# mit-acl/dpgo_ros

Measured on AMD Instinct MI355X. Metric: ms/RBCD-iteration + iterations-to-1e-6-relcost, sphere2500 5-agent, lower is better.
Workload: dtype f64; 1 GPU; sphere2500.g2o, 5 agents, synchronous round-robin RBCD, RGD(step 0.2, dense preconditioner) + Nesterov (restart 20), r=5, library weighting; mid-run iterations one launch each (k_step_fd: the private part of an agent's preconditioner product formed by the launch before its own, its row products by the one before that), hipGraphs of up to 256 iterations; agents=5, poses_per_agent=500, placement=agent a on rank a % N

## Files before the change

dpgo_ros_amd/csrc/device_math.h:

```cpp
#pragma once
#include <hip/hip_runtime.h>

namespace dpgo {

typedef double v2d_t __attribute__((ext_vector_type(2)));

template <class T>
__device__ __forceinline__ __attribute__((address_space(1))) T *gp(T *p) { return (__attribute__((address_space(1))) T *)p; }

__device__ __forceinline__ void sym3_eig(const double S[9], double w[3], double V[9]) {
  double A[9];
#pragma unroll
  for (int i = 0; i < 9; ++i) { A[i] = S[i]; V[i] = (i % 4 == 0) ? 1.0 : 0.0; }
  for (int sweep = 0; sweep < 12; ++sweep) {
    const double off = A[1] * A[1] + A[2] * A[2] + A[5] * A[5];
    const double dia = A[0] * A[0] + A[4] * A[4] + A[8] * A[8];
    if (off <= 1e-32 * dia) break;
#pragma unroll
    for (int p = 0; p < 2; ++p) {
#pragma unroll
      for (int q = p + 1; q < 3; ++q) {
        const double apq = A[3 * p + q];
        if (apq != 0.0) {
          const double theta = (A[4 * q] - A[4 * p]) / (2.0 * apq);
// ... 289 lines not shown
    }
#pragma unroll
  for (int i = 0; i < 3 * R; ++i) W[i] = T[i];
}

template <int R>
__device__ __forceinline__ void tangent_row(const double *Yp, const double *Wp, int a, double out[3]) {
  double S[9];
#pragma unroll
  for (int p = 0; p < 3; ++p)
#pragma unroll
    for (int q = 0; q < 3; ++q) {
      double s = 0;
#pragma unroll
      for (int b = 0; b < R; ++b) s += Yp[p * R + b] * Wp[q * R + b];
      S[3 * p + q] = s;
    }
#pragma unroll
  for (int q = 0; q < 3; ++q) {
    double s = Wp[q * R + a];
#pragma unroll
    for (int p = 0; p < 3; ++p) s -= Yp[p * R + a] * 0.5 * (S[3 * p + q] + S[3 * q + p]);
    out[q] = s;
  }
}

__device__ __forceinline__ void lanes_sync() {
  __builtin_amdgcn_fence(__ATOMIC_RELEASE, "wavefront");
  __builtin_amdgcn_wave_barrier();
  __builtin_amdgcn_fence(__ATOMIC_ACQUIRE, "wavefront");
}

template <int R>
__device__ __forceinline__ void gram3_lanes(const double *A, double *S, int s) {
  if (s < 6) {
    const int i = (s < 3) ? 0 : ((s < 5) ? 1 : 2), j = (s < 3) ? s : ((s < 5) ? s - 2 : 2);
    double acc = 0;
#pragma unroll
    for (int a = 0; a < R; ++a) acc += A[i * R + a] * A[j * R + a];
    S[3 * i + j] = acc;
    S[3 * j + i] = acc;
  }
  lanes_sync();
}

template <int R>
__device__ __forceinline__ void polar_lanes(double *A, double *S, int s) {
  gram3_lanes<R>(A, S, s);
  double e0 = 1.0 - S[0], e1 = 1.0 - S[4], e2 = 1.0 - S[8];
  double dev = e0 * e0 + e1 * e1 + e2 * e2 + 2.0 * (S[1] * S[1] + S[2] * S[2] + S[5] * S[5]);
  if (!(dev < 0.1)) {
    lanes_sync();
    if (s == 0) {
      double a[3 * R];
#pragma unroll
      for (int i = 0; i < 3 * R; ++i) a[i] = A[i];
      polar_inplace<R>(a);
#pragma unroll
      for (int i = 0; i < 3 * R; ++i) A[i] = a[i];
    }
    lanes_sync();
    return;
  }
  double d = dev;
  const int j = (s < 3 * R) ? s / R : 0, a = (s < 3 * R) ? s - j * R : 0;
#pragma unroll 1
  for (int it = 0; it < 8 && d > 1e-31; ++it) {
    double T[3];
#pragma unroll
    for (int k = 0; k < 3; ++k) T[k] = -0.5 * S[3 * k + j];
    if (j == 0) T[0] += 1.5;
    if (j == 1) T[1] += 1.5;
    if (j == 2) T[2] += 1.5;
    const double b = A[a] * T[0] + A[R + a] * T[1] + A[2 * R + a] * T[2];
    lanes_sync();
    if (s < 3 * R) A[s] = b;
    lanes_sync();
    if (d * d <= 1e-31) break;
    gram3_lanes<R>(A, S, s);
    const double f0 = 1.0 - S[0], f1 = 1.0 - S[4], f2 = 1.0 - S[8];
    d = f0 * f0 + f1 * f1 + f2 * f2 + 2.0 * (S[1] * S[1] + S[2] * S[2] + S[5] * S[5]);
  }
}

template <int R>
__device__ __forceinline__ void qf_lanes(double *A, double *G, int s) {
  if (s < 6) {
    const int i = (s < 3) ? 0 : ((s < 5) ? 1 : 2), j = (s < 3) ? s : ((s < 5) ? s - 2 : 2);
    double acc = 0;
#pragma unroll
    for (int a = 0; a < R; ++a) acc += A[i * R + a] * A[j * R + a];
    G[s] = acc;
  }
  lanes_sync();
  const double g00 = G[0], g01 = G[1], g02 = G[2], g11 = G[3], g12 = G[4], g22 = G[5];
  const double e0 = 1.0 - g00, e1 = 1.0 - g11, e2 = 1.0 - g22;
  const double dev = e0 * e0 + e1 * e1 + e2 * e2 + 2.0 * (g01 * g01 + g02 * g02 + g12 * g12);
  if (dev < 0.05) {
    const double i0 = rsqrt(g00);
    const double r01 = g01 * i0, r02 = g02 * i0;
    const double i1 = rsqrt(g11 - r01 * r01);
    const double r12 = (g12 - r01 * r02) * i1;
    const double i2 = rsqrt(g22 - r02 * r02 - r12 * r12);
    if (s < R) {
      const int a = s;
      const double q0 = A[a] * i0;
      const double q1 = (A[R + a] - r01 * q0) * i1;
      const double q2 = (A[2 * R + a] - r02 * q0 - r12 * q1) * i2;
      A[a] = q0; A[R + a] = q1; A[2 * R + a] = q2;
    }
    lanes_sync();
    return;
  }
  if (s == 0) {
    double a[3 * R];
#pragma unroll
    for (int i = 0; i < 3 * R; ++i) a[i] = A[i];
    qf_inplace<R>(a);
#pragma unroll
    for (int i = 0; i < 3 * R; ++i) A[i] = a[i];
  }
  lanes_sync();
}

template <int R>
__device__ __forceinline__ void tangent_lanes(const double *Y, double *W, double *S, int s) {
  if (s < 9) {
    const int p = s / 3, q = s - 3 * p;
    double acc = 0;
#pragma unroll
    for (int a = 0; a < R; ++a) acc += Y[p * R + a] * W[q * R + a];
    S[3 * p + q] = acc;
  }
  lanes_sync();
  double t = 0;
  if (s < 3 * R) {
    const int q = s / R, a = s - q * R;
    t = W[q * R + a];
#pragma unroll
    for (int p = 0; p < 3; ++p) t -= Y[p * R + a] * 0.5 * (S[3 * p + q] + S[3 * q + p]);
  }
  lanes_sync();
  if (s < 3 * R) W[s] = t;
  lanes_sync();
}

template <int CTRL>
__device__ __forceinline__ double dpp_move(double v) {
  int lo = __double2loint(v), hi = __double2hiint(v);
  lo = __builtin_amdgcn_update_dpp(0, lo, CTRL, 0xF, 0xF, true);
  hi = __builtin_amdgcn_update_dpp(0, hi, CTRL, 0xF, 0xF, true);
  return __hiloint2double(hi, lo);
}
__device__ __forceinline__ double wave_sum(double x) {
  x += dpp_move<0xB1>(x);
  x += dpp_move<0x4E>(x);
  x += dpp_move<0x141>(x);
  x += dpp_move<0x140>(x);
  const int lo = __double2loint(x), hi = __double2hiint(x);
  double r[4];
#pragma unroll
  for (int q = 0; q < 4; ++q)
    r[q] = __hiloint2double(__builtin_amdgcn_readlane(hi, 16 * q), __builtin_amdgcn_readlane(lo, 16 * q));
  return (r[0] + r[1]) + (r[2] + r[3]);
}

__device__ __forceinline__ double sum_partials(const double *p, int count, int stride, int lane) {
  double s = 0;
  for (int base = 0; base < count; base += 512) {
    double v[8];
#pragma unroll
    for (int u = 0; u < 8; ++u) {
      const int i = base + lane + 64 * u;
      v[u] = (i < count) ? gp(p)[(size_t)i * stride] : 0.0;
    }
#pragma unroll
    for (int u = 0; u < 8; ++u) s += v[u];
  }
  return wave_sum(s);
}

__device__ __forceinline__ void sum_partials2(const double *p, int count, int stride, int lane, double &s0, double &s1) {
  double a = 0, b = 0;
  for (int base = 0; base < count; base += 512) {
    double2 v[8];
#pragma unroll
    for (int u = 0; u < 8; ++u) {
      const int i = base + lane + 64 * u;
      if (i < count) { const v2d_t t = *(const __attribute__((address_space(1))) v2d_t *)(p + (size_t)i * stride); v[u] = make_double2(t.x, t.y); } else v[u] = make_double2(0.0, 0.0);
    }
#pragma unroll
    for (int u = 0; u < 8; ++u) { a += v[u].x; b += v[u].y; }
  }
  s0 = wave_sum(a);
  s1 = wave_sum(b);
}

}
```

dpgo_ros_amd/csrc/step_deep.hip:

```cpp
#include "kernel_common.h"
#include <algorithm>

namespace dpgo {

constexpr int FD_KC = 2048;
#ifndef DPGO_FD_HEAD
#define DPGO_FD_HEAD 0
#endif
#ifndef DPGO_FD_GC_LATE
#define DPGO_FD_GC_LATE 0
#endif
#ifndef DPGO_FD_PACC_WT
#define DPGO_FD_PACC_WT 0
#endif
#ifndef DPGO_FD_E_EARLY
#define DPGO_FD_E_EARLY 0
#endif
#ifndef DPGO_FD_KA_PREFETCH
#define DPGO_FD_KA_PREFETCH 1
#endif
constexpr int FD_HEAD = DPGO_FD_HEAD;

enum { FD_SY_C = 0, FD_SY_E, FD_SY_D, FD_SY_F, FD_SY_N, FD_SY_RQ, FD_SY_COUNT = 8 };

__device__ __forceinline__ void fd_signal(int *cnt) {
  __builtin_amdgcn_fence(__ATOMIC_RELEASE, "workgroup", "local");
  if ((threadIdx.x & 63) == 0) __hip_atomic_fetch_add(cnt, 1, __ATOMIC_RELAXED, __HIP_MEMORY_SCOPE_WORKGROUP);
}

__device__ __forceinline__ void fd_signal_requested(int *cnt) {
  __builtin_amdgcn_sched_barrier(0);
  asm volatile("" ::: "memory");
  if ((threadIdx.x & 63) == 0) __hip_atomic_fetch_add(cnt, 1, __ATOMIC_RELAXED, __HIP_MEMORY_SCOPE_WORKGROUP);
  asm volatile("" ::: "memory");
  __builtin_amdgcn_sched_barrier(0);
}

__device__ __forceinline__ void fd_wait(int *cnt, int target) {
  for (int spin = 0; spin < (1 << 22) && __hip_atomic_load(cnt, __ATOMIC_RELAXED, __HIP_MEMORY_SCOPE_WORKGROUP) < target; ++spin)
    __builtin_amdgcn_s_sleep(1);
  __builtin_amdgcn_fence(__ATOMIC_ACQUIRE, "workgroup", "local");
}

template <int R>
__device__ __forceinline__ int fd_pos_off(const unsigned char *ord, int pose) {
  const int ch = pose >> 4;
  int p = 0;
#pragma unroll
  for (int i = 0; i < 32; ++i) p = ((int)ord[i] == ch) ? i : p;
  return p * 64 * R + (pose & 15) * 4 * R;
}

template <int R>
struct FdXn {
  double2 v[3][2 * R];
};

template <int R>
__device__ __forceinline__ void fd_xn_request(const AgentDev &ag, const FeBases &fb, int parity, int ln, FdXn<R> &xr) {
#pragma unroll
  for (int q = 0; q < 3; ++q) {
    {
      unsigned wsel = 0;
#pragma unroll
      for (int k = 0; k < 32; ++k) {
        const unsigned wk = ag.fe_code[(32 * q + k < FE_MAX_EDGES / 2) ? 32 * q + k : FE_MAX_EDGES / 2 - 1];
        wsel = ((ln >> 1) == k) ? wk : wsel;
      }
      const unsigned code = (ln & 1) ? (wsel >> 16) : (wsel & 0xffffu);
      const int sa = (int)(code >> 12), sf = (int)(code & 0xfffu);
      const double *yb = fb.ybase[0];
      int yn = fb.npose[0];
#pragma unroll
      for (int k = 1; k < LOOKAHEAD_MAX_AGENTS; ++k) { yb = (sa == k) ? fb.ybase[k] : yb; yn = (sa == k) ? fb.npose[k] : yn; }
      const double *xp = yb + (parity ? (size_t)B_ALT * 4 * R * yn : (size_t)0) + (size_t)sf * 4 * R;
#pragma unroll
      for (int k = 0; k < 2 * R; ++k) xr.v[q][k] = ld2(xp + 2 * k);
    }
  }
}

template <int R>
__device__ __forceinline__ void fd_xn_to_lds(const AgentDev &ag, int ln, const FdXn<R> &xr, double *Es) {
  constexpr int EPE = 4 * R + 16;
  int nsh = ag.nshared;
  asm volatile("" : "+v"(nsh));
#pragma unroll
  for (int q = 0; q < 3; ++q) {
    if (64 * q < nsh && 64 * q + ln < nsh) {
      double *E = Es + (size_t)(64 * q + ln) * EPE;
#pragma unroll
      for (int k = 0; k < 2 * R; ++k) *reinterpret_cast<double2 *>(E + 2 * k) = xr.v[q][k];
    }
  }
}

struct FdCf {
  static constexpr int TRIPS = FE_MAX_EDGES * 8 / 64;
  double2 v[TRIPS];
};

__device__ __forceinline__ void fd_cf_request(const AgentDev &ag, int ln, FdCf &cr) {
  const int nit = ag.nshared * 8;
#pragma unroll
  for (int j = 0; j < FdCf::TRIPS; ++j) cr.v[j] = ld2(ag.fe_coef + 2 * min(64 * j + ln, nit - 1));
}

template <int R>
__device__ __forceinline__ void fd_cf_to_lds(const AgentDev &ag, int ln, const FdCf &cr, double *Es) {
  constexpr int EPE = 4 * R + 16;
  int nit = ag.nshared * 8;
  asm volatile("" : "+v"(nit));
#pragma unroll
  for (int j = 0; j < FdCf::TRIPS; ++j) {
    const int t = 64 * j + ln;
    if (64 * j < nit && t < nit) *reinterpret_cast<double2 *>(Es + (size_t)(t >> 3) * EPE + 4 * R + 2 * (t & 7)) = cr.v[j];
  }
}

struct FdNest {
  bool restart_now, restart_next, restart_next2, restart_next3;
  double nest_gamma, ahead_alpha, ahead2_alpha, ahead3_alpha;
};

__device__ __forceinline__ FdNest fd_nest(const NestState &ns, int num_robots, int restart_interval) {
  FdNest o;
  const double Nr = (double)num_robots;
  o.restart_now = ((ns.iter + 2) % restart_interval) == 0;
  o.restart_next = ((ns.iter + 3) % restart_interval) == 0;
  o.restart_next2 = ((ns.iter + 4) % restart_interval) == 0;
  o.restart_next3 = ((ns.iter + 5) % restart_interval) == 0;
  o.nest_gamma = o.restart_now ? 0.0 : (1.0 + sqrt(1.0 + 4.0 * Nr * Nr * ns.gamma * ns.gamma)) / (2.0 * Nr);
  const double g2 = (1.0 + sqrt(1.0 + 4.0 * Nr * Nr * o.nest_gamma * o.nest_gamma)) / (2.0 * Nr);
  o.ahead_alpha = 1.0 / (g2 * Nr);
  const double gamma_next = o.restart_next ? 0.0 : g2;
  const double g3 = (1.0 + sqrt(1.0 + 4.0 * Nr * Nr * gamma_next * gamma_next)) / (2.0 * Nr);
  o.ahead2_alpha = 1.0 / (g3 * Nr);
  const double gamma_next2 = o.restart_next2 ? 0.0 : g3;
  const double g4 = (1.0 + sqrt(1.0 + 4.0 * Nr * Nr * gamma_next2 * gamma_next2)) / (2.0 * Nr);
  o.ahead3_alpha = 1.0 / (g4 * Nr);
  return o;
}

template <int R, int NC>
struct FdCur {
  double2 mc[NC];
  double pa[R];
};

template <int R, int M0, int NC>
__device__ __forceinline__ void fd_cur_request(const AgentDev &ag, const double *pacc_in, int bx, int nblk, int l, FdCur<R, NC> &cu) {
  const int cg = (l >> 5) & 7, kl = l & 31;
  const int N4 = ag.N4, col = 8 * bx + cg;
  const double *Mc = ag.M + (size_t)((col < N4) ? col : 0) * N4;
#pragma unroll
  for (int i = 0; i < NC; ++i) cu.mc[i] = ld2_nt(Mc + min(2 * kl + 64 * (int)ag.fe_ord[M0 + i], N4 - 2));
#pragma unroll
  for (int a = 0; a < R; ++a) cu.pa[a] = gp(pacc_in)[((size_t)min(bx, nblk - 1) * R + a) * 256 + l];
}

template <int R, int M0, int NC>
__device__ __forceinline__ void fd_cur_product(const FdCur<R, NC> &cu, const double *vs, double *red, int l) {
  const int cg = (l >> 5) & 7, kl = l & 31;
  double acc[R];
#pragma unroll
  for (int a = 0; a < R; ++a) acc[a] = cu.pa[a];
#pragma unroll
  for (int i = 0; i < NC; ++i) {
    const int k = 2 * kl + 64 * (M0 + i);
    double wv[2 * R];
#pragma unroll
    for (int q = 0; q < R; ++q) {
      const double2 t2 = *reinterpret_cast<const double2 *>(&vs[k * R + 2 * q]);
      wv[2 * q] = t2.x; wv[2 * q + 1] = t2.y;
    }
#pragma unroll
    for (int a = 0; a < R; ++a) acc[a] = __builtin_fma(wv[R + a], cu.mc[i].y, __builtin_fma(wv[a], cu.mc[i].x, acc[a]));
  }
#pragma unroll
  for (int a = 0; a < R; ++a) red[kl * (8 * R + 1) + cg * R + a] = acc[a];
}

#ifdef DPGO_FE_TRACE
#ifndef DPGO_FE_TRACE_BLOCK
#define DPGO_FE_TRACE_BLOCK 100
#endif
#define FD_TRACE_DECL __shared__ unsigned long long fd_stamps[8 * 16];
#ifndef DPGO_FD_STAMP_MASK
#define DPGO_FD_STAMP_MASK 0xFFFF
#endif
#define FD_STAMP(k) do { if (((DPGO_FD_STAMP_MASK >> (k)) & 1) && (threadIdx.x & 63) == 0) fd_stamps[(threadIdx.x >> 6) * 16 + (k)] = wall_clock64(); } while (0)
#define FD_FLUSH() do { if ((threadIdx.x & 63) == 0) { const int w_ = threadIdx.x >> 6; \
    if (blockIdx.x == DPGO_FE_TRACE_BLOCK) for (int k_ = 0; k_ < 16; ++k_) ag.part[PART_E + 4000 * PART_STRIDE + w_ * 16 + k_] = (double)fd_stamps[w_ * 16 + k_]; \
    if (w_ == 4) { ag.part[PART_E + (4100 + 2 * (int)blockIdx.x) * PART_STRIDE] = (double)fd_stamps[4 * 16]; ag.part[PART_E + (4100 + 2 * (int)blockIdx.x) * PART_STRIDE + 1] = (double)fd_stamps[4 * 16 + 15]; } \
    if (w_ == 0) { ag.part[PART_E + (4100 + 2 * (int)blockIdx.x) * PART_STRIDE + 2] = (double)fd_stamps[15]; } } } while (0)
#elif defined(DPGO_FD_ENDS)
#define FD_TRACE_DECL
#define FD_STAMP(k) do { if ((k) == 0 && blockIdx.x == 100 && threadIdx.x == 256) ag.part[PART_E + 4000 * PART_STRIDE + 64] = (double)wall_clock64(); } while (0)
#define FD_FLUSH() do { if (blockIdx.x == 100 && (threadIdx.x & 63) == 0) ag.part[PART_E + 4000 * PART_STRIDE + (threadIdx.x >> 6) * 16 + 15] = (double)wall_clock64(); } while (0)
#else
#define FD_TRACE_DECL
#define FD_STAMP(k) do { } while (0)
#define FD_FLUSH() do { } while (0)
#endif

template <int R, int M0>
__global__ __launch_bounds__(512) void k_step_fd(TeamDev *team, int sel, int next_sel, double step, int num_robots, int restart_interval,
                                                 const NestState *nest_src, NestState *nest_dst, int parity, const AgentDev agv,
                                                 int next3_sel, int flags, const FdNext nx, const FeBases fb,
                                                 const double *__restrict__ pacc_in, double *__restrict__ pacc_out, int nblk_all,
                                                 int num_agents) {
  const AgentDev &ag = agv;
#if DPGO_FD_KA_PREFETCH
  {
    const unsigned *ka = (const unsigned *)__builtin_amdgcn_kernarg_segment_ptr();
    constexpr int KA_LINES = (int)((sizeof(AgentDev) + sizeof(FdNext) + sizeof(FeBases) + 160 + 63) / 64);
    unsigned touch = 0;
#pragma unroll
    for (int i = 0; i < KA_LINES; ++i) touch |= ka[16 * i];
    asm volatile("" ::"s"(touch));
  }
#endif
  const double *__restrict__ Xr = ag.buf[parity ? B_XALT : B_X];
  const double *__restrict__ Yr = ag.buf[parity ? B_YALT : B_Y];
  double *__restrict__ Xw = ag.buf[parity ? B_X : B_XALT];
  double *__restrict__ Yw = ag.buf[parity ? B_Y : B_YALT];
  const int hb = (int)blockIdx.x;
  const int bx = (hb % 8) * ((int)gridDim.x / 8) + hb / 8;
  const int tid = threadIdx.x;
  const int N4 = ag.N4, n = ag.n;
  const int nblk = (N4 + 7) / 8;
  if (bx >= nblk_all) return;
  const bool own = bx < nblk, in = (flags & FD_IN) != 0;
  constexpr int KC = FD_KC, MREG = KC / 64, NC = MREG - M0;
  __shared__ double vs[R * KC];
  __shared__ double zs[8 * R];
  __shared__ double red[32 * (8 * R + 1)];
  __shared__ double Ysh[2 * 4 * R];
  __shared__ double Esh[2][2 * 4 * R];
  __shared__ double Es[FE_MAX_EDGES * (4 * R + 16)];
  __shared__ double tl_x[2 * 4 * R], tl_v[2 * 4 * R], tl_y[2 * 4 * R], tl_s[2 * 16];
  __shared__ double Ex[2 * 3 * 4 * R];
  __shared__ double Psh[2 * 4 * R], tl_rel[2];
  __shared__ int sy[FD_SY_COUNT];
  FD_TRACE_DECL
  FD_STAMP(0);
  if (tid < FD_SY_COUNT) sy[tid] = 0;
  lds_barrier();
  const int pj0 = own ? 2 * bx : 0, pj1 = (own && 2 * bx + 1 < n) ? 2 * bx + 1 : -1;
  const int npose = own ? ((pj1 >= 0) ? 2 : 1) : 0;
  constexpr int EPE = 4 * R + 16;
  const int cwv = __builtin_amdgcn_readfirstlane(tid >> 6), ln = tid & 63;

  if (cwv < 4) {
    const int cg = (tid >> 5) & 7, kl = tid & 31;
    for (int t = N4 * R + tid; t < KC * R; t += 256) vs[t] = 0.0;
    constexpr int NGC = ((KC - 64 * M0) * R / 2 + 255) / 256;
    double2 gc[NGC];
#if !DPGO_FD_GC_LATE
    {
      const double *Gc = ag.buf[B_CARRY_G];
#pragma unroll
      for (int u = 0; u < NGC; ++u) gc[u] = ld2(Gc + min(M0 * 64 * R + 2 * (tid + 256 * u), N4 * R - 2));
    }
#endif
    const int cold = 8 * bx + cg;
    const int N4d = nx.N4d;
    const double *Md = nx.Md + (size_t)((cold < N4d) ? cold : 0) * N4d;
    double2 mn[M0];
#pragma unroll
    for (int i = 0; i < FD_HEAD; ++i) mn[i] = ld2_nt(Md + min(2 * kl + 64 * (int)nx.ord_d[i], N4d - 2));
    FD_STAMP(10);
    __builtin_amdgcn_sched_barrier(0);
#if DPGO_FD_GC_LATE
    {
      const double *Gc = ag.buf[B_CARRY_G];
#pragma unroll
      for (int u = 0; u < NGC; ++u) gc[u] = ld2(Gc + min(M0 * 64 * R + 2 * (tid + 256 * u), N4 * R - 2));
    }
#endif
#pragma unroll
    for (int u = 0; u < NGC; ++u) {
      const int tt = M0 * 64 * R + 2 * (tid + 256 * u);
      if (tt < N4 * R) *reinterpret_cast<double2 *>(&vs[tt]) = gc[u];
    }
    fd_signal(&sy[FD_SY_C]);
    FD_STAMP(1);
    fd_wait(&sy[FD_SY_RQ], 4);
    FD_STAMP(11);
    __builtin_amdgcn_sched_barrier(0);
    asm volatile("" ::: "memory");
    constexpr int NGN = (M0 * 64 * R / 2 + 255) / 256;
    double2 gn[NGN];
#pragma unroll
    for (int u = 0; u < NGN; ++u) gn[u] = ld2(nx.Gd + min(2 * (tid + 256 * u), M0 * 64 * R - 2));
#pragma unroll
    for (int i = FD_HEAD; i < M0; ++i) mn[i] = ld2_nt(Md + min(2 * kl + 64 * (int)nx.ord_d[i], N4d - 2));
    FD_STAMP(12);
#pragma unroll
    for (int u = 0; u < NGN; ++u) {
      const int tt = 2 * (tid + 256 * u);
      if (tt < M0 * 64 * R) *reinterpret_cast<double2 *>(&vs[tt]) = gn[u];
    }
    fd_signal(&sy[FD_SY_N]);
    fd_wait(&sy[FD_SY_N], 4);
    fd_wait(&sy[FD_SY_F], 4);
    FD_STAMP(13);
    double acc[R];
#pragma unroll
    for (int a = 0; a < R; ++a) acc[a] = 0;
#pragma unroll
    for (int i = 0; i < M0; ++i) {
      const int k = 2 * kl + 64 * i;
      double wv[2 * R];
#pragma unroll
      for (int q = 0; q < R; ++q) {
        const double2 t2 = *reinterpret_cast<const double2 *>(&vs[k * R + 2 * q]);
        wv[2 * q] = t2.x; wv[2 * q + 1] = t2.y;
      }
#pragma unroll
      for (int a = 0; a < R; ++a) acc[a] = __builtin_fma(wv[R + a], mn[i].y, __builtin_fma(wv[a], mn[i].x, acc[a]));
    }
    if ((flags & FD_P) && bx < nx.nblk_d) {
#pragma unroll
#if DPGO_FD_PACC_WT
      for (int a = 0; a < R; ++a) st_c(pacc_out + ((size_t)bx * R + a) * 256 + tid, acc[a]);
#else
      for (int a = 0; a < R; ++a) gp(pacc_out)[((size_t)bx * R + a) * 256 + tid] = acc[a];
#endif
    }
    FD_STAMP(15);
    FD_FLUSH();
    return;
  }

  if (cwv < 6) {
    const int g = cwv - 4;
    const int npub = ag.npub;
    const int pq = 64 * g + ln;
    const bool pact = pq < npub;
    const int pqc = pact ? pq : 0;
    const int pj = ag.pub_pose[pqc];
    const int pe0 = ag.pub_ptr[pqc], pe1 = ag.pub_ptr[pqc + (pact ? 1 : 0)];
    double w[4 * R], x[4 * R];
    {
      const double *Wc = ag.buf[B_CARRY_W], *Xc = ag.buf[B_CARRY_X];
#pragma unroll
      for (int i = 0; i < 2 * R; ++i) {
        const double2 tw = ld2(Wc + ((size_t)i * npub + pqc) * 2), tx = ld2(Xc + ((size_t)i * npub + pqc) * 2);
        w[2 * i] = tw.x; w[2 * i + 1] = tw.y; x[2 * i] = tx.x; x[2 * i + 1] = tx.y;
      }
    }
    FD_STAMP(14);
    FdCur<R, NC> cu;
    fd_cur_request<R, M0, NC>(ag, pacc_in, bx, nblk, tid - 256, cu);
    const int npw = (nx.n_e + nblk_all - 1) / nblk_all;
    const int wls = ln / (4 * R), we = ln - wls * (4 * R);
    const int pw = bx * npw + wls;
    const bool pv = wls < 3 && wls < npw && pw < nx.n_e;
    const int pwc = pv ? pw : 0;
    const int wtile = pwc >> 6, wpl = pwc & 63, wdn = nx.soa_w_e;
    int ii[8];
#pragma unroll
    for (int u = 0; u < 8; ++u) ii[u] = gp(nx.soa_col_e)[((size_t)wtile * wdn + min(u, wdn - 1)) * 64 + wpl];
    const int qi = gp(nx.pub_index_e)[pwc];
    const int tl = tid - 256 - 64 * g;
    const size_t own_off = (size_t)((tl >= 4 * R) ? max(pj1, 0) : pj0) * 4 * R + (size_t)(tl % (4 * R));
    double pre_x = 0, pre_v = 0, pre_y = 0, pre_p = 0;
    if (tl < npose * 4 * R) {
      pre_x = gp(Xr)[own_off];
      pre_v = gp(ag.buf[B_V])[own_off];
      pre_y = gp(Yr)[own_off];
      pre_p = gp(ag.buf[B_XPREV])[own_off];
    }
    const NestState ns = nest_src[sel];
    __builtin_amdgcn_s_setprio(3);
    FD_STAMP(10);
    fd_signal_requested(&sy[FD_SY_RQ]);
    FD_STAMP(11);
    const int vs_off = fd_pos_off<R>(ag.fe_ord, pj);
    fd_wait(&sy[FD_SY_E], 2);
    FD_STAMP(1);
    if (pact) {
      double gg[4 * R];
#pragma unroll
      for (int i = 0; i < 4 * R; ++i) gg[i] = 0.0;
      for (int e = pe0; e < pe1; ++e) {
        const double *E = Es + (size_t)e * EPE;
        double xn[4 * R];
#pragma unroll
        for (int i = 0; i < 2 * R; ++i) { const double2 t = *reinterpret_cast<const double2 *>(E + 2 * i); xn[2 * i] = t.x; xn[2 * i + 1] = t.y; }
#pragma unroll
        for (int c = 0; c < 4; ++c) {
          const double2 c01 = *reinterpret_cast<const double2 *>(E + 4 * R + 4 * c), c23 = *reinterpret_cast<const double2 *>(E + 4 * R + 4 * c + 2);
          const double cfc[4] = {c01.x, c01.y, c23.x, c23.y};
#pragma unroll
          for (int cp = 0; cp < 4; ++cp)
#pragma unroll
            for (int a = 0; a < R; ++a) gg[c * R + a] -= xn[cp * R + a] * cfc[cp];
        }
      }
#pragma unroll
      for (int i = 0; i < 4 * R; ++i) w[i] = w[i] + gg[i];
      tangent_inplace<R>(x, w);
    }
    FD_STAMP(3);
    fd_wait(&sy[FD_SY_C], 4);
    FD_STAMP(2);
    if (pact) {
#pragma unroll
      for (int i = 0; i < 4 * R; ++i) vs[vs_off + i] = w[i];
    }
    FD_STAMP(12);
    fd_signal(&sy[FD_SY_D]);
    FD_STAMP(13);
    fd_wait(&sy[FD_SY_D], 2);
    FD_STAMP(4);
    fd_cur_product<R, M0, NC>(cu, vs, red, tid - 256);
    if (tl >= 0 && tl < npose * 4 * R) { Ysh[tl] = pre_x; Esh[0][tl] = pre_v; Esh[1][tl] = pre_y; Psh[tl] = pre_p; }
    FD_STAMP(5);
    fd_signal(&sy[FD_SY_F]);
    if (g == 1) {
      __builtin_amdgcn_s_setprio(0);
      const int c = we / R, a = we - c * R;
      const double *__restrict__ Y2 = nx.Ye;
      double xv[8][4], bv[8][4];
#pragma unroll
      for (int u = 0; u < 8; ++u) {
        const double *xp = Y2 + (size_t)4 * R * ii[u] + a;
        const double *bp = nx.soa_val_e + ((size_t)wtile * wdn + min(u, wdn - 1)) * 1024 + (2 * c) * 128 + 2 * wpl;
        xv[u][0] = gp(xp)[0]; xv[u][1] = gp(xp)[R]; xv[u][2] = gp(xp)[2 * R]; xv[u][3] = gp(xp)[3 * R];
        bv[u][0] = gp(bp)[0]; bv[u][1] = gp(bp)[1]; bv[u][2] = gp(bp)[128]; bv[u][3] = gp(bp)[129];
      }
      const double xe_ = gp(Y2)[(size_t)4 * R * pwc + we];
      double acc = 0.0;
#pragma unroll
      for (int u = 0; u < 8; ++u) {
        const double t = fma4(xv[u][0], bv[u][0], xv[u][1], bv[u][1], xv[u][2], bv[u][2], xv[u][3], bv[u][3], acc);
        acc = (u < wdn) ? t : acc;
      }
      const bool wr = pv && (flags & FD_W);
      if (wr && qi >= 0) {
        gp(nx.We)[((size_t)(we >> 1) * nx.npub_e + qi) * 2 + (we & 1)] = acc;
        gp(nx.Xe)[((size_t)(we >> 1) * nx.npub_e + qi) * 2 + (we & 1)] = xe_;
      }
      if (wls < 3) { Ex[wls * 4 * R + we] = acc; Ex[3 * 4 * R + wls * 4 * R + we] = xe_; }
      WSYNC();
      if (wr && we == 0) {
        double ww[4 * R], xx[4 * R];
#pragma unroll
        for (int i = 0; i < 4 * R; ++i) { ww[i] = Ex[wls * 4 * R + i]; xx[i] = Ex[3 * 4 * R + wls * 4 * R + i]; }
        tangent_inplace<R>(xx, ww);
        double *Gn = nx.Ge + fd_pos_off<R>(nx.ord_e, pw);
#pragma unroll
        for (int i = 0; i < 4 * R; ++i) gp(Gn)[i] = ww[i];
      }
      FD_STAMP(14);
      FD_FLUSH();
      return;
    }
    fd_wait(&sy[FD_SY_F], 4);
    if (ln < 8 * R) {
      double s = 0;
#pragma unroll
      for (int q = 0; q < 32; ++q) s += red[q * (8 * R + 1) + ln];
      zs[ln] = s;
    }
    FD_STAMP(6);
    WSYNC();
    const FdNest nn = fd_nest(ns, num_robots, restart_interval);
    const bool restart_now = nn.restart_now, restart_next = nn.restart_next;
    const double nest_gamma = nn.nest_gamma, ahead_alpha = nn.ahead_alpha;
    const bool ahead_opt = next_sel == sel;
    const bool stats = in && (flags & FD_STATS) != 0, lastat = in && (flags & FD_LASTAT) != 0;
    if (ln < 2) tl_rel[ln] = 0.0;
    {
      const int lp = ln >> 4, s = ln & 15;
      if (lp < npose) {
        const size_t o = (size_t)(lp ? pj1 : pj0) * 4 * R;
        double *xs = tl_x + lp * 4 * R, *vsv = tl_v + lp * 4 * R, *ys = tl_y + lp * 4 * R, *Ss = tl_s + lp * 16;
        double *zz = zs + lp * 4 * R;
        const double *x0 = Ysh + lp * 4 * R, *v0 = Esh[0] + lp * 4 * R, *y0 = Esh[1] + lp * 4 * R;
        const int i0 = s, i1 = s + 16;
        const bool h0 = i0 < 4 * R, h1 = i1 < 4 * R;
        tangent_lanes<R>(x0, zz, Ss, s);
        if (h0) xs[i0] = x0[i0] - step * zz[i0];
        if (h1) xs[i1] = x0[i1] - step * zz[i1];
        lanes_sync();
        qf_lanes<R>(xs, Ss, s);
        FD_STAMP(7);
        if (stats) {
          if (h0) gp(ag.buf[B_X2])[o + i0] = xs[i0];
          if (h1) gp(ag.buf[B_X2])[o + i1] = xs[i1];
          if (s == 0) {
            const double *p0 = Psh + lp * 4 * R;
            double rel = 0;
#pragma unroll
            for (int i = 0; i < 4 * R; ++i) { const double d = xs[i] - p0[i]; rel += d * d; }
            tl_rel[lp] = rel;
          }
        }
        if (lastat) {
          if (h0) gp(ag.buf[B_XPREV])[o + i0] = xs[i0];
          if (h1) gp(ag.buf[B_XPREV])[o + i1] = xs[i1];
        }
        const bool reset = restart_now;
        if (reset) {
          if (h0) vsv[i0] = xs[i0];
          if (h1) vsv[i1] = xs[i1];
          lanes_sync();
        } else {
          const double gamma = nest_gamma;
          if (h0) vsv[i0] = v0[i0] + gamma * (xs[i0] - y0[i0]);
          if (h1) vsv[i1] = v0[i1] + gamma * (xs[i1] - y0[i1]);
          lanes_sync();
          polar_lanes<R>(vsv, Ss, s);
        }
        FD_STAMP(8);
        if (restart_next) {
          if (h0 && in) {
            Xw[o + i0] = xs[i0];
            if (!ahead_opt) { Yw[o + i0] = xs[i0]; vsv[i0] = xs[i0]; }
            else Yw[o + i0] = reset ? xs[i0] : y0[i0];
          }
          if (h1 && in) {
            Xw[o + i1] = xs[i1];
            if (!ahead_opt) { Yw[o + i1] = xs[i1]; vsv[i1] = xs[i1]; }
            else Yw[o + i1] = reset ? xs[i1] : y0[i1];
          }
          if (lastat && !ahead_opt && s == 0) gp(ag.part)[PART_D + (lp ? pj1 : pj0)] = 0.0;
        } else {
          if (h0) ys[i0] = (1.0 - ahead_alpha) * xs[i0] + ahead_alpha * vsv[i0];
          if (h1) ys[i1] = (1.0 - ahead_alpha) * xs[i1] + ahead_alpha * vsv[i1];
          lanes_sync();
          polar_lanes<R>(ys, Ss, s);
          FD_STAMP(9);
          if (h0 && in) { Yw[o + i0] = ys[i0]; Xw[o + i0] = ys[i0]; }
          if (h1 && in) { Yw[o + i1] = ys[i1]; Xw[o + i1] = ys[i1]; }
          if (lastat && !ahead_opt && s == 0) {
            double rel2 = 0;
#pragma unroll
            for (int i = 0; i < 4 * R; ++i) { const double d = ys[i] - xs[i]; rel2 += d * d; }
            gp(ag.part)[PART_D + (lp ? pj1 : pj0)] = rel2;
          }
        }
        lanes_sync();
        if (h0 && in) ag.buf[B_V][o + i0] = vsv[i0];
        if (h1 && in) ag.buf[B_V][o + i1] = vsv[i1];
      }
    }
    if (stats) {
      WSYNC();
      double rl = (ln < npose) ? tl_rel[ln] : 0.0;
      rl = wave_sum(rl);
      if (ln == 0 && own) gp(ag.part)[PART_B + (size_t)bx * PART_STRIDE + 2] = rl;
    }
    FD_STAMP(15);
    FD_FLUSH();
    return;
  }

  const int h = cwv - 6;
  if (h == 0) {
    FdXn<R> er;
    fd_xn_request<R>(ag, fb, parity, ln, er);
    FD_STAMP(9);
    FdCur<R, NC> cu;
    fd_cur_request<R, M0, NC>(ag, pacc_in, bx, nblk, tid - 256, cu);
    FD_STAMP(10);
    fd_signal_requested(&sy[FD_SY_RQ]);
    FD_STAMP(11);
    __builtin_amdgcn_s_setprio(3);
    fd_xn_to_lds<R>(ag, ln, er, Es);
    fd_signal(&sy[FD_SY_E]);
    FD_STAMP(8);
    fd_wait(&sy[FD_SY_D], 2);
    fd_cur_product<R, M0, NC>(cu, vs, red, tid - 256);
    fd_signal(&sy[FD_SY_F]);
    if (bx == 0 && ln < LOOKAHEAD_MAX_AGENTS && in) {
      const int k = ln;
      const double Nr = (double)num_robots;
      if (k < num_agents) {
        NestState s2 = nest_src[k];
        const bool restart = ((s2.iter + 2) % restart_interval) == 0;
        if (restart) { s2.gamma = 0; s2.alpha = 0; }
        else {
          s2.gamma = (1.0 + sqrt(1.0 + 4.0 * Nr * Nr * s2.gamma * s2.gamma)) / (2.0 * Nr);
          s2.alpha = 1.0 / (s2.gamma * Nr);
        }
        s2.iter += 1;
        nest_dst[k] = s2;
      }
      if (k == 0) {
        team->iter += 1;
        team->stats_sel = sel;
        team->next_sel = next_sel;
        team->cur_sel = next_sel;
      }
    }
    FD_STAMP(14);
    FD_FLUSH();
    return;
  }

  {
    FdCf er;
    fd_cf_request(ag, ln, er);
    FD_STAMP(9);
    FdCur<R, NC> cu;
    fd_cur_request<R, M0, NC>(ag, pacc_in, bx, nblk, tid - 256, cu);
#if DPGO_FD_E_EARLY
    __builtin_amdgcn_sched_barrier(0);
    fd_cf_to_lds<R>(ag, ln, er, Es);
    fd_signal(&sy[FD_SY_E]);
    FD_STAMP(8);
    __builtin_amdgcn_sched_barrier(0);
#endif
    int pre[LOOKAHEAD_MAX_AGENTS + 1];
    pre[0] = 0;
#pragma unroll
    for (int k = 0; k < LOOKAHEAD_MAX_AGENTS; ++k) pre[k + 1] = pre[k] + ((k < num_agents) ? fb.npose[k] : 0);
    const int total = pre[LOOKAHEAD_MAX_AGENTS] - n;
    const int per = (total + nblk_all - 1) / nblk_all;
    const int q = bx * per + ln;
    const bool lact = ln < per && q < total;
    int self_lo = 0;
#pragma unroll
    for (int k = 0; k < LOOKAHEAD_MAX_AGENTS; ++k) if (k == sel) self_lo = pre[k];
    const int gq = lact ? (q < self_lo ? q : q + n) : 0;
    int a = 0, lo = 0, na_ = fb.npose[0];
    const double *ya = fb.ybase[0];
#pragma unroll
    for (int k = 1; k < LOOKAHEAD_MAX_AGENTS; ++k)
      if (k < num_agents && gq >= pre[k]) { a = k; lo = pre[k]; ya = fb.ybase[k]; na_ = fb.npose[k]; }
    const size_t vlen = (size_t)4 * R * na_;
    double *yp = const_cast<double *>(ya);
    double *xa = yp - (size_t)(B_Y - B_X) * vlen, *va = yp + (size_t)(B_V - B_Y) * vlen;
    const size_t da = (size_t)B_ALT * vlen;
    const double *xr = parity ? xa + da : xa, *yr = parity ? yp + da : yp;
    double *oX = parity ? xa : xa + da, *oY = parity ? yp : yp + da, *oV = va;
    const int la_pose = gq - lo;
    const bool la_opt = next_sel == a;
    const size_t o = (size_t)la_pose * 4 * R;
    double la_x[4 * R], la_v[4 * R];
#pragma unroll
    for (int i = 0; i < 2 * R; ++i) {
      const double2 tx = ld2(xr + o + 2 * i), tv = ld2(va + o + 2 * i);
      la_x[2 * i] = tx.x; la_x[2 * i + 1] = tx.y; la_v[2 * i] = tv.x; la_v[2 * i + 1] = tv.y;
    }
    const NestState ns = nest_src[sel];
    FD_STAMP(10);
    fd_signal_requested(&sy[FD_SY_RQ]);
    FD_STAMP(11);
    __builtin_amdgcn_s_setprio(3);
#if !DPGO_FD_E_EARLY
    fd_cf_to_lds<R>(ag, ln, er, Es);
    fd_signal(&sy[FD_SY_E]);
    FD_STAMP(8);
#endif
    fd_wait(&sy[FD_SY_D], 2);
    fd_cur_product<R, M0, NC>(cu, vs, red, tid - 256);
    fd_signal(&sy[FD_SY_F]);
    __builtin_amdgcn_s_setprio(0);
    const FdNest nn = fd_nest(ns, num_robots, restart_interval);
    if (lact) {
      const bool st = in, lastat = in && (flags & FD_LASTAT) != 0;
      double *pa_ = fb.part[0];
#pragma unroll
      for (int k = 1; k < LOOKAHEAD_MAX_AGENTS; ++k) pa_ = (a == k) ? fb.part[k] : pa_;
      if (lastat) {
        double *xprev = yp - (size_t)(B_Y - B_XPREV) * vlen;
#pragma unroll
        for (int i = 0; i < 4 * R; ++i) gp(xprev)[o + i] = la_x[i];
      }
      if (nn.restart_next) {
#pragma unroll
        for (int i = 0; i < 4 * R; ++i) {
          if (st) oX[o + i] = la_x[i];
          if (!la_opt) { if (st) { oY[o + i] = la_x[i]; oV[o + i] = la_x[i]; } la_v[i] = la_x[i]; }
          else if (st) oY[o + i] = yr[o + i];
        }
        if (lastat && !la_opt) gp(pa_)[PART_D + la_pose] = 0.0;
      } else {
        double y[4 * R];
#pragma unroll
        for (int i = 0; i < 4 * R; ++i) y[i] = (1.0 - nn.ahead_alpha) * la_x[i] + nn.ahead_alpha * la_v[i];
        polar_inplace<R>(y);
        if (lastat && !la_opt) {
          double r2 = 0;
#pragma unroll
          for (int i = 0; i < 4 * R; ++i) { const double d = y[i] - la_x[i]; r2 += d * d; }
          gp(pa_)[PART_D + la_pose] = r2;
        }
#pragma unroll
        for (int i = 0; i < 4 * R; ++i) { if (st) { oY[o + i] = y[i]; oX[o + i] = y[i]; } la_x[i] = y[i]; }
      }
      FD_STAMP(7);
      if ((flags & FD_Y) && a == next3_sel) {
        if (nn.restart_next2) {
#pragma unroll
          for (int i = 0; i < 4 * R; ++i) la_v[i] = la_x[i];
        } else {
          double y[4 * R];
#pragma unroll
          for (int i = 0; i < 4 * R; ++i) y[i] = (1.0 - nn.ahead2_alpha) * la_x[i] + nn.ahead2_alpha * la_v[i];
          polar_inplace<R>(y);
#pragma unroll
          for (int i = 0; i < 4 * R; ++i) la_x[i] = y[i];
        }
        if (!nn.restart_next3) {
          double y[4 * R];
#pragma unroll
          for (int i = 0; i < 4 * R; ++i) y[i] = (1.0 - nn.ahead3_alpha) * la_x[i] + nn.ahead3_alpha * la_v[i];
          polar_inplace<R>(y);
#pragma unroll
          for (int i = 0; i < 4 * R; ++i) la_x[i] = y[i];
        }
        double *py3 = yp + (size_t)(B_CARRY_Y - B_Y) * (long long)vlen;
#pragma unroll
        for (int i = 0; i < 4 * R; ++i) gp(py3)[o + i] = la_x[i];
      }
    }
    FD_STAMP(15);
    FD_FLUSH();
  }
}

template <int R>
__global__ __launch_bounds__(64) void k_fd_prime(const AgentDev *__restrict__ agents, int s0, int s1, int s2, int num_robots,
                                                 int restart_interval, const NestState *nest_src) {
  const int role = (int)blockIdx.y;
  const int ai = role == 0 ? s0 : (role == 1 ? s1 : s2);
  const AgentDev &ag = agents[ai];
  const int j = (int)blockIdx.x * 64 + (int)threadIdx.x;
  if (j >= ag.n) return;
  const size_t o = (size_t)j * 4 * R;
  double x[4 * R], v[4 * R];
#pragma unroll
  for (int i = 0; i < 4 * R; ++i) { x[i] = gp(ag.buf[B_X])[o + i]; v[i] = gp(ag.buf[B_V])[o + i]; }
  const FdNest nn = fd_nest(nest_src[s0], num_robots, restart_interval);
  if (role == 2) {
    if (nn.restart_next) {
#pragma unroll
      for (int i = 0; i < 4 * R; ++i) v[i] = x[i];
    } else {
      double y[4 * R];
#pragma unroll
      for (int i = 0; i < 4 * R; ++i) y[i] = (1.0 - nn.ahead_alpha) * x[i] + nn.ahead_alpha * v[i];
      polar_inplace<R>(y);
#pragma unroll
      for (int i = 0; i < 4 * R; ++i) x[i] = y[i];
    }
  }
  if (role >= 1) {
    const bool rs = role == 1 ? nn.restart_next : nn.restart_next2;
    const double al = role == 1 ? nn.ahead_alpha : nn.ahead2_alpha;
    if (!rs) {
      double y[4 * R];
#pragma unroll
      for (int i = 0; i < 4 * R; ++i) y[i] = (1.0 - al) * x[i] + al * v[i];
      polar_inplace<R>(y);
#pragma unroll
      for (int i = 0; i < 4 * R; ++i) x[i] = y[i];
    }
  }
#pragma unroll
  for (int i = 0; i < 4 * R; ++i) gp(ag.buf[B_CARRY_Y])[o + i] = x[i];
}

template <int R>
__global__ __launch_bounds__(64) void k_fd_rows(const AgentDev *__restrict__ agents, int e0, int e1, int nblk_all) {
  const AgentDev &age = agents[blockIdx.y == 0 ? e0 : e1];
  const int bx = (int)blockIdx.x, ln = (int)threadIdx.x;
  __shared__ double Ex[2 * 3 * 4 * R];
  const int npw = (age.n + nblk_all - 1) / nblk_all;
  const int wls = ln / (4 * R), we = ln - wls * (4 * R);
  const int pw = bx * npw + wls;
  const bool pv = wls < 3 && wls < npw && pw < age.n;
  const int pwc = pv ? pw : 0;
  const int wtile = pwc >> 6, wpl = pwc & 63, wdn = age.soa_w;
  int ii[8];
#pragma unroll
  for (int u = 0; u < 8; ++u) ii[u] = gp(age.soa_col)[((size_t)wtile * wdn + min(u, wdn - 1)) * 64 + wpl];
  const int qi = gp(age.pub_index)[pwc];
  const int c = we / R, a = we - c * R;
  const double *__restrict__ Y2 = age.buf[B_CARRY_Y];
  double xv[8][4], bv[8][4];
#pragma unroll
  for (int u = 0; u < 8; ++u) {
    const double *xp = Y2 + (size_t)4 * R * ii[u] + a;
    const double *bp = age.soa_val + ((size_t)wtile * wdn + min(u, wdn - 1)) * 1024 + (2 * c) * 128 + 2 * wpl;
    xv[u][0] = gp(xp)[0]; xv[u][1] = gp(xp)[R]; xv[u][2] = gp(xp)[2 * R]; xv[u][3] = gp(xp)[3 * R];
    bv[u][0] = gp(bp)[0]; bv[u][1] = gp(bp)[1]; bv[u][2] = gp(bp)[128]; bv[u][3] = gp(bp)[129];
  }
  const double xe_ = gp(Y2)[(size_t)4 * R * pwc + we];
  double acc = 0.0;
#pragma unroll
  for (int u = 0; u < 8; ++u) {
    const double t = fma4(xv[u][0], bv[u][0], xv[u][1], bv[u][1], xv[u][2], bv[u][2], xv[u][3], bv[u][3], acc);
    acc = (u < wdn) ? t : acc;
  }
  if (pv && qi >= 0) {
    gp(age.buf[B_CARRY_W])[((size_t)(we >> 1) * age.npub + qi) * 2 + (we & 1)] = acc;
    gp(age.buf[B_CARRY_X])[((size_t)(we >> 1) * age.npub + qi) * 2 + (we & 1)] = xe_;
  }
  if (wls < 3) { Ex[wls * 4 * R + we] = acc; Ex[3 * 4 * R + wls * 4 * R + we] = xe_; }
  WSYNC();
  if (pv && we == 0) {
    double ww[4 * R], xx[4 * R];
#pragma unroll
    for (int i = 0; i < 4 * R; ++i) { ww[i] = Ex[wls * 4 * R + i]; xx[i] = Ex[3 * 4 * R + wls * 4 * R + i]; }
    tangent_inplace<R>(xx, ww);
    double *Gn = age.buf[B_CARRY_G] + fd_pos_off<R>(age.fe_ord, pw);
// ... 111 lines not shown
```

Measured before the change: 12.90 us.

## Split public-pose row work across four waves using lane pairs per pose

Public-pose gradient and tangent projection work moves from two waves (one lane per pose, full 4R rows) to four waves, where each pose is handled by a lane pair, each lane owning half the columns. DPP swaps exchange point data, edge ranges and the symmetric-part terms, so per-lane register and compute load is halved and the two waves that used to just wait now do useful work. The lookahead wave's x/v loads are deferred until after the public-row phase to cut register pressure. The cost is extra cross-lane shuffles, a four-wave barrier instead of two, and later issue of the lookahead loads.

```diff
diff --git a/dpgo_ros_amd/csrc/device_math.h b/dpgo_ros_amd/csrc/device_math.h
--- a/dpgo_ros_amd/csrc/device_math.h
+++ b/dpgo_ros_amd/csrc/device_math.h
@@ -465,6 +465,38 @@
   hi = __builtin_amdgcn_update_dpp(0, hi, CTRL, 0xF, 0xF, true);
   return __hiloint2double(hi, lo);
 }
+template <int R>
+__device__ __forceinline__ void tangent_pair(const double *Y, double *Wh, bool hi) {
+  double s[3][2];
+#pragma unroll
+  for (int p = 0; p < 3; ++p)
+#pragma unroll
+    for (int cc = 0; cc < 2; ++cc) {
+      double t = 0;
+#pragma unroll
+      for (int a = 0; a < R; ++a) t += Y[p * R + a] * Wh[cc * R + a];
+      s[p][cc] = t;
+    }
+  const double r0 = dpp_move<0xB1>(hi ? s[0][0] : s[2][0]);
+  const double r1 = dpp_move<0xB1>(hi ? s[1][0] : s[2][1]);
+  double T[2 * R];
+#pragma unroll
+  for (int cc = 0; cc < 2; ++cc) {
+    const double Sc[3] = {s[0][cc], s[1][cc], s[2][cc]};
+    const double Sr[3] = {cc == 0 ? (hi ? r0 : s[0][0]) : s[1][0], cc == 0 ? (hi ? r1 : s[0][1]) : s[1][1],
+                          cc == 0 ? (hi ? s[2][0] : r0) : r1};
+#pragma unroll
+    for (int a = 0; a < R; ++a) {
+      double t = Wh[cc * R + a];
+#pragma unroll
+      for (int p = 0; p < 3; ++p) t -= Y[p * R + a] * 0.5 * (Sc[p] + Sr[p]);
+      T[cc * R + a] = t;
+    }
+  }
+#pragma unroll
+  for (int a = 0; a < R; ++a) { Wh[a] = T[a]; Wh[R + a] = hi ? Wh[R + a] : T[R + a]; }
+}
+
 __device__ __forceinline__ double wave_sum(double x) {
   x += dpp_move<0xB1>(x);
   x += dpp_move<0x4E>(x);
diff --git a/dpgo_ros_amd/csrc/step_deep.hip b/dpgo_ros_amd/csrc/step_deep.hip
--- a/dpgo_ros_amd/csrc/step_deep.hip
+++ b/dpgo_ros_amd/csrc/step_deep.hip
@@ -116,6 +116,74 @@
     const int t = 64 * j + ln;
     if (64 * j < nit && t < nit) *reinterpret_cast<double2 *>(Es + (size_t)(t >> 3) * EPE + 4 * R + 2 * (t & 7)) = cr.v[j];
   }
+}
+
+constexpr int FD_PUB_WAVES = 4;
+
+template <int R>
+struct FdPub {
+  static constexpr int NXP = (3 * R + 1) / 2;
+  static constexpr int HX = (NXP + 1) / 2;
+  double2 w[R], x[HX];
+  int pe, pj;
+  bool pact;
+};
+
+template <int R>
+__device__ __forceinline__ void fd_pub_request(const AgentDev &ag, int pw, int ln, FdPub<R> &pb) {
+  const int npub = ag.npub, hi = ln & 1;
+  const int pq = 32 * pw + (ln >> 1);
+  pb.pact = pq < npub;
+  const int pqc = pb.pact ? pq : 0;
+  pb.pj = ag.pub_pose[pqc];
+  pb.pe = ag.pub_ptr[pqc + ((hi && pb.pact) ? 1 : 0)];
+  const double *Wc = ag.buf[B_CARRY_W], *Xc = ag.buf[B_CARRY_X];
+#pragma unroll
+  for (int k = 0; k < R; ++k) pb.w[k] = ld2(Wc + ((size_t)(hi * R + k) * npub + pqc) * 2);
+#pragma unroll
+  for (int k = 0; k < FdPub<R>::HX; ++k) pb.x[k] = ld2(Xc + ((size_t)min(hi * FdPub<R>::HX + k, FdPub<R>::NXP - 1) * npub + pqc) * 2);
+}
+
+template <int R>
+__device__ __forceinline__ void fd_pub_point(const FdPub<R> &pb, bool hi, double *x, int &pe0, int &pe1) {
+  constexpr int NXP = FdPub<R>::NXP, HX = FdPub<R>::HX;
+  const int po = __builtin_amdgcn_update_dpp(0, pb.pe, 0xB1, 0xF, 0xF, true);
+  pe0 = hi ? po : pb.pe;
+  pe1 = hi ? pb.pe : po;
+#pragma unroll
+  for (int k = 0; k < HX; ++k) {
+    const double ox = pb.x[k].x, oy = pb.x[k].y;
+    const double sx = dpp_move<0xB1>(ox), sy_ = dpp_move<0xB1>(oy);
+    x[2 * k] = hi ? sx : ox; x[2 * k + 1] = hi ? sy_ : oy;
+    if (HX + k < NXP) { x[2 * (HX + k)] = hi ? ox : sx; x[2 * (HX + k) + 1] = hi ? oy : sy_; }
+  }
+}
+
+template <int R>
+__device__ __forceinline__ void fd_pub_gradient(int pe0, int pe1, const double *x, const double *Es, bool hi, double *wl) {
+  constexpr int EPE = 4 * R + 16;
+  double gg[2 * R];
+#pragma unroll
+  for (int i = 0; i < 2 * R; ++i) gg[i] = 0.0;
+  for (int e = pe0; e < pe1; ++e) {
+    const double *E = Es + (size_t)e * EPE;
+    double xn[4 * R];
+#pragma unroll
+    for (int i = 0; i < 2 * R; ++i) { const double2 t = *reinterpret_cast<const double2 *>(E + 2 * i); xn[2 * i] = t.x; xn[2 * i + 1] = t.y; }
+    const double *Ec = E + 4 * R + (hi ? 8 : 0);
+#pragma unroll
+    for (int cc = 0; cc < 2; ++cc) {
+      const double2 c01 = *reinterpret_cast<const double2 *>(Ec + 4 * cc), c23 = *reinterpret_cast<const double2 *>(Ec + 4 * cc + 2);
+      const double cfc[4] = {c01.x, c01.y, c23.x, c23.y};
+#pragma unroll
+      for (int cp = 0; cp < 4; ++cp)
+#pragma unroll
+        for (int a = 0; a < R; ++a) gg[cc * R + a] -= xn[cp * R + a] * cfc[cp];
+    }
+  }
+#pragma unroll
+  for (int i = 0; i < 2 * R; ++i) wl[i] = wl[i] + gg[i];
+  tangent_pair<R>(x, wl, hi);
 }
 
 struct FdNest {
@@ -249,8 +317,32 @@
   lds_barrier();
   const int pj0 = own ? 2 * bx : 0, pj1 = (own && 2 * bx + 1 < n) ? 2 * bx + 1 : -1;
   const int npose = own ? ((pj1 >= 0) ? 2 : 1) : 0;
-  constexpr int EPE = 4 * R + 16;
   const int cwv = __builtin_amdgcn_readfirstlane(tid >> 6), ln = tid & 63;
+
+  auto pub_rows = [&](const FdPub<R> &pb) __attribute__((always_inline)) {
+    const bool hi = (ln & 1) != 0;
+    const int vs_off = fd_pos_off<R>(ag.fe_ord, pb.pj) + (hi ? 2 * R : 0);
+    double x[2 * FdPub<R>::NXP], wl[2 * R];
+    int pe0, pe1;
+    fd_pub_point<R>(pb, hi, x, pe0, pe1);
+#pragma unroll
+    for (int k = 0; k < R; ++k) { wl[2 * k] = pb.w[k].x; wl[2 * k + 1] = pb.w[k].y; }
+    fd_wait(&sy[FD_SY_E], 2);
+    FD_STAMP(1);
+    if (pb.pact) fd_pub_gradient<R>(pe0, pe1, x, Es, hi, wl);
+    FD_STAMP(3);
+    fd_wait(&sy[FD_SY_C], 4);
+    FD_STAMP(2);
+    if (pb.pact) {
+#pragma unroll
+      for (int i = 0; i < 2 * R; ++i) vs[vs_off + i] = wl[i];
+    }
+    FD_STAMP(12);
+    fd_signal(&sy[FD_SY_D]);
+    FD_STAMP(13);
+    fd_wait(&sy[FD_SY_D], FD_PUB_WAVES);
+    FD_STAMP(4);
+  };
 
   if (cwv < 4) {
     const int cg = (tid >> 5) & 7, kl = tid & 31;
@@ -336,21 +428,8 @@
 
   if (cwv < 6) {
     const int g = cwv - 4;
-    const int npub = ag.npub;
-    const int pq = 64 * g + ln;
-    const bool pact = pq < npub;
-    const int pqc = pact ? pq : 0;
-    const int pj = ag.pub_pose[pqc];
-    const int pe0 = ag.pub_ptr[pqc], pe1 = ag.pub_ptr[pqc + (pact ? 1 : 0)];
-    double w[4 * R], x[4 * R];
-    {
-      const double *Wc = ag.buf[B_CARRY_W], *Xc = ag.buf[B_CARRY_X];
-#pragma unroll
-      for (int i = 0; i < 2 * R; ++i) {
-        const double2 tw = ld2(Wc + ((size_t)i * npub + pqc) * 2), tx = ld2(Xc + ((size_t)i * npub + pqc) * 2);
-        w[2 * i] = tw.x; w[2 * i + 1] = tw.y; x[2 * i] = tx.x; x[2 * i + 1] = tx.y;
-      }
-    }
+    FdPub<R> pb;
+    fd_pub_request<R>(ag, g, ln, pb);
     FD_STAMP(14);
     FdCur<R, NC> cu;
     fd_cur_request<R, M0, NC>(ag, pacc_in, bx, nblk, tid - 256, cu);
@@ -378,44 +457,7 @@
     FD_STAMP(10);
     fd_signal_requested(&sy[FD_SY_RQ]);
     FD_STAMP(11);
-    const int vs_off = fd_pos_off<R>(ag.fe_ord, pj);
-    fd_wait(&sy[FD_SY_E], 2);
-    FD_STAMP(1);
-    if (pact) {
-      double gg[4 * R];
-#pragma unroll
-      for (int i = 0; i < 4 * R; ++i) gg[i] = 0.0;
-      for (int e = pe0; e < pe1; ++e) {
-        const double *E = Es + (size_t)e * EPE;
-        double xn[4 * R];
-#pragma unroll
-        for (int i = 0; i < 2 * R; ++i) { const double2 t = *reinterpret_cast<const double2 *>(E + 2 * i); xn[2 * i] = t.x; xn[2 * i + 1] = t.y; }
-#pragma unroll
-        for (int c = 0; c < 4; ++c) {
-          const double2 c01 = *reinterpret_cast<const double2 *>(E + 4 * R + 4 * c), c23 = *reinterpret_cast<const double2 *>(E + 4 * R + 4 * c + 2);
-          const double cfc[4] = {c01.x, c01.y, c23.x, c23.y};
-#pragma unroll
-          for (int cp = 0; cp < 4; ++cp)
-#pragma unroll
-            for (int a = 0; a < R; ++a) gg[c * R + a] -= xn[cp * R + a] * cfc[cp];
-        }
-      }
-#pragma unroll
-      for (int i = 0; i < 4 * R; ++i) w[i] = w[i] + gg[i];
-      tangent_inplace<R>(x, w);
-    }
-    FD_STAMP(3);
-    fd_wait(&sy[FD_SY_C], 4);
-    FD_STAMP(2);
-    if (pact) {
-#pragma unroll
-      for (int i = 0; i < 4 * R; ++i) vs[vs_off + i] = w[i];
-    }
-    FD_STAMP(12);
-    fd_signal(&sy[FD_SY_D]);
-    FD_STAMP(13);
-    fd_wait(&sy[FD_SY_D], 2);
-    FD_STAMP(4);
+    pub_rows(pb);
     fd_cur_product<R, M0, NC>(cu, vs, red, tid - 256);
     if (tl >= 0 && tl < npose * 4 * R) { Ysh[tl] = pre_x; Esh[0][tl] = pre_v; Esh[1][tl] = pre_y; Psh[tl] = pre_p; }
     FD_STAMP(5);
@@ -565,6 +607,8 @@
     FdXn<R> er;
     fd_xn_request<R>(ag, fb, parity, ln, er);
     FD_STAMP(9);
+    FdPub<R> pb;
+    fd_pub_request<R>(ag, 2, ln, pb);
     FdCur<R, NC> cu;
     fd_cur_request<R, M0, NC>(ag, pacc_in, bx, nblk, tid - 256, cu);
     FD_STAMP(10);
@@ -574,7 +618,7 @@
     fd_xn_to_lds<R>(ag, ln, er, Es);
     fd_signal(&sy[FD_SY_E]);
     FD_STAMP(8);
-    fd_wait(&sy[FD_SY_D], 2);
+    pub_rows(pb);
     fd_cur_product<R, M0, NC>(cu, vs, red, tid - 256);
     fd_signal(&sy[FD_SY_F]);
     if (bx == 0 && ln < LOOKAHEAD_MAX_AGENTS && in) {
@@ -607,6 +651,8 @@
     FdCf er;
     fd_cf_request(ag, ln, er);
     FD_STAMP(9);
+    FdPub<R> pb;
+    fd_pub_request<R>(ag, 3, ln, pb);
     FdCur<R, NC> cu;
     fd_cur_request<R, M0, NC>(ag, pacc_in, bx, nblk, tid - 256, cu);
 #if DPGO_FD_E_EARLY
@@ -642,12 +688,6 @@
     const int la_pose = gq - lo;
     const bool la_opt = next_sel == a;
     const size_t o = (size_t)la_pose * 4 * R;
-    double la_x[4 * R], la_v[4 * R];
-#pragma unroll
-    for (int i = 0; i < 2 * R; ++i) {
-      const double2 tx = ld2(xr + o + 2 * i), tv = ld2(va + o + 2 * i);
-      la_x[2 * i] = tx.x; la_x[2 * i + 1] = tx.y; la_v[2 * i] = tv.x; la_v[2 * i + 1] = tv.y;
-    }
     const NestState ns = nest_src[sel];
     FD_STAMP(10);
     fd_signal_requested(&sy[FD_SY_RQ]);
@@ -658,7 +698,14 @@
     fd_signal(&sy[FD_SY_E]);
     FD_STAMP(8);
 #endif
-    fd_wait(&sy[FD_SY_D], 2);
+    pub_rows(pb);
+    __builtin_amdgcn_sched_barrier(0);
+    double la_x[4 * R], la_v[4 * R];
+#pragma unroll
+    for (int i = 0; i < 2 * R; ++i) {
+      const double2 tx = ld2(xr + o + 2 * i), tv = ld2(va + o + 2 * i);
+      la_x[2 * i] = tx.x; la_x[2 * i + 1] = tx.y; la_v[2 * i] = tv.x; la_v[2 * i + 1] = tv.y;
+    }
     fd_cur_product<R, M0, NC>(cu, vs, red, tid - 256);
     fd_signal(&sy[FD_SY_F]);
     __builtin_amdgcn_s_setprio(0);
```

Result: slower. 13.54 us (+5.0%).
